# dfm/tinygp

Measured on AMD Instinct MI355X. Metric: GP log_probability evals/sec + Cholesky TFLOP/s (fp64), N=16,384, higher is better.
Workload: dtype f64; 1 GPU; c2: 1.5^2 ExpSquared(2.5), 1-D X, N=16384, fp64, diag=0.01, constant-density synthetic inputs (SURVEY 8d), dense Cholesky + tri-solve; n=16384, d=1, parallelism=single, nb_outer=1024

## Files before the change

tinygp_amd/csrc/capi.hip:

```cpp
#include <cmath>
#include <cstdlib>
#include <chrono>
#include <cstring>
#include <string>

#include "tgp_common.h"
#define CHAIN_HD __host__ __device__
#include "chain_tasks.h"
#define TILE_HD
#include "tile_order.h"

namespace tgp {

static thread_local std::string g_error;

void set_error(const char* fmt, ...) {
  char buf[1024];
  va_list ap;
  va_start(ap, fmt);
  vsnprintf(buf, sizeof(buf), fmt, ap);
  va_end(ap);
  g_error = buf;
}

// ... 147 lines not shown
    const char* b = getenv("TGP_SERIALIZED_KERNELS");
    auto on = [](const char* v) { return v != nullptr && *v && strcmp(v, "0") != 0 && strcasecmp(v, "false") != 0; };
    if (on(a) || on(b)) {
      ctx->serializing_tool = true;
      ctx->chain_polls = 0;
    }
  }
  TGP_HIP_TRY(hipStreamCreateWithPriority(&ctx->panel_stream, hipStreamNonBlocking, hi));
  TGP_HIP_TRY(hipStreamCreateWithPriority(&ctx->update_stream, hipStreamNonBlocking, hi));
  TGP_HIP_TRY(hipStreamCreateWithPriority(&ctx->asm_stream, hipStreamNonBlocking, lo));
  TGP_HIP_TRY(hipEventCreateWithFlags(&ctx->ev_asm, hipEventDisableTiming));
  TGP_HIP_TRY(hipEventCreateWithFlags(&ctx->ev_d, hipEventDisableTiming));
  TGP_HIP_TRY(hipEventCreateWithFlags(&ctx->ev_e, hipEventDisableTiming));
  TGP_HIP_TRY(hipEventCreateWithFlags(&ctx->ev_f, hipEventDisableTiming));
  TGP_HIP_TRY(hipEventCreateWithFlags(&ctx->ev_g1, hipEventDisableTiming));
  TGP_HIP_TRY(hipEventCreateWithFlags(&ctx->ev_g2, hipEventDisableTiming));
  TGP_HIP_TRY(hipEventCreateWithFlags(&ctx->ev_h, hipEventDisableTiming));
  TGP_HIP_TRY(hipEventCreateWithFlags(&ctx->ev_i, hipEventDisableTiming));
  TGP_HIP_TRY(hipEventCreateWithFlags(&ctx->ev_j, hipEventDisableTiming));
  TGP_HIP_TRY(hipEventCreateWithFlags(&ctx->ev_c, hipEventDisableTiming));
  TGP_HIP_TRY(hipEventCreateWithFlags(&ctx->ev_join, hipEventDisableTiming));
  TGP_HIP_TRY(hipEventCreateWithFlags(&ctx->ev_a, hipEventDisableTiming));
  TGP_HIP_TRY(hipEventCreateWithFlags(&ctx->ev_b, hipEventDisableTiming));
  TGP_HIP_TRY(hipMalloc(&ctx->d_scal, 16 * sizeof(double)));
  TGP_HIP_TRY(hipMalloc(&ctx->d_info, sizeof(int32_t)));
  TGP_HIP_TRY(hipMalloc(&ctx->d_step_flag, 64));
  TGP_HIP_TRY(hipMemset(ctx->d_step_flag, 0, 64));
  TGP_HIP_TRY(hipMalloc(&ctx->d_chain_flags, size_t(tgp::CHAIN_MAX_ROW_TILES) * 64 * sizeof(uint32_t)));
  TGP_HIP_TRY(hipMemset(ctx->d_chain_flags, 0, size_t(tgp::CHAIN_MAX_ROW_TILES) * 64 * sizeof(uint32_t)));
  TGP_HIP_TRY(hipMalloc(&ctx->d_chain_ticket, 4096));
  TGP_HIP_TRY(hipMemset(ctx->d_chain_ticket, 0, 4096));
  TGP_HIP_TRY(hipMalloc(&ctx->d_chain_red, size_t(2) * CHAIN_MAX_ROW_TILES * sizeof(double)));
  hipDeviceProp_t prop;
  TGP_HIP_TRY(hipGetDeviceProperties(&prop, device));
  ctx->cus = prop.multiProcessorCount;
  *out = ctx;
  return TGP_OK;
}

int tgp_ctx_destroy(tgp_ctx* ctx) {
  if (!ctx) return TGP_OK;
  hipSetDevice(ctx->device);
  hipStreamSynchronize(ctx->stream);
  if (ctx->panel_stream) hipStreamSynchronize(ctx->panel_stream);
  if (ctx->solve_stream) {
    hipStreamSynchronize(ctx->solve_stream);
    hipStreamDestroy(ctx->solve_stream);
  }
  if (ctx->ev_c) hipEventDestroy(ctx->ev_c);
  if (ctx->ev_join) hipEventDestroy(ctx->ev_join);
  if (ctx->ev_asm_gate) hipEventDestroy(ctx->ev_asm_gate);
  if (ctx->rescue_stream) hipStreamDestroy(ctx->rescue_stream);
  if (ctx->update_stream) {
    hipStreamSynchronize(ctx->update_stream);
    hipStreamDestroy(ctx->update_stream);
  }
  if (ctx->asm_stream) {
    hipStreamSynchronize(ctx->asm_stream);
    hipStreamDestroy(ctx->asm_stream);
  }
  if (ctx->ev_asm) hipEventDestroy(ctx->ev_asm);
  if (ctx->ev_d) hipEventDestroy(ctx->ev_d);
  if (ctx->ev_e) hipEventDestroy(ctx->ev_e);
  if (ctx->ev_f) hipEventDestroy(ctx->ev_f);
  if (ctx->ev_g1) hipEventDestroy(ctx->ev_g1);
  if (ctx->ev_g2) hipEventDestroy(ctx->ev_g2);
  if (ctx->ev_h) hipEventDestroy(ctx->ev_h);
  if (ctx->ev_i) hipEventDestroy(ctx->ev_i);
  if (ctx->ev_j) hipEventDestroy(ctx->ev_j);
  for (auto e : ctx->ev_pool) hipEventDestroy(e);
  if (ctx->ev_a) hipEventDestroy(ctx->ev_a);
  if (ctx->ev_b) hipEventDestroy(ctx->ev_b);
  if (ctx->d_scal) hipFree(ctx->d_scal);
  if (ctx->d_info) hipFree(ctx->d_info);
  if (ctx->d_step_flag) hipFree(ctx->d_step_flag);
  if (ctx->d_chain_flags) hipFree(ctx->d_chain_flags);
  if (ctx->d_chain_ticket) hipFree(ctx->d_chain_ticket);
  if (ctx->d_chain_red) hipFree(ctx->d_chain_red);
  if (ctx->d_chain_stamps) hipFree(ctx->d_chain_stamps);
  for (auto& kv : ctx->chain_tables)
    if (kv.second.dev) hipFree(kv.second.dev);
  if (ctx->d_dinv) hipFree(ctx->d_dinv);
  if (ctx->d_work) hipFree(ctx->d_work);
  if (ctx->d_gemm_ws) hipFree(ctx->d_gemm_ws);
  if (ctx->panel_stream) hipStreamDestroy(ctx->panel_stream);
  if (ctx->own_stream && ctx->stream) hipStreamDestroy(ctx->stream);
  delete ctx;
  return TGP_OK;
}

int tgp_ctx_sync(tgp_ctx* ctx) {
  CTX_GUARD(ctx);
  TGP_HIP_TRY(hipStreamSynchronize(ctx->stream));
  return TGP_OK;
}

static int64_t* option_slot(tgp_ctx* ctx, const char* key) {
// ... 39 lines not shown
  if (!strcmp(key, "host_join")) return &ctx->host_join;
  if (!strcmp(key, "late_join")) return &ctx->late_join;
  if (!strcmp(key, "chain_reduce")) return &ctx->chain_reduce;
  if (!strcmp(key, "asm_defer")) return &ctx->asm_defer;
  if (!strcmp(key, "tile_band")) return &ctx->tile_band;
  if (!strcmp(key, "fault_inject")) return &ctx->fault_inject;
  if (!strcmp(key, "poll_timeout_ms")) return &ctx->poll_timeout_ms;
  if (!strcmp(key, "timeout_retries")) return &ctx->timeout_retries;
  return nullptr;
}

static int set_option_checked(tgp_ctx* ctx, const char* key, int64_t value, int64_t* old) {
  int64_t* slot = option_slot(ctx, key);
  TGP_ARG_CHECK(slot != nullptr, "unknown option '%s'", key);
  if (slot == &ctx->nb_outer)
    TGP_ARG_CHECK(value >= TILE && value % TILE == 0, "nb_outer must be a positive multiple of %d", TILE);
  if (slot == &ctx->sub_panel || slot == &ctx->nb_first)
    TGP_ARG_CHECK(value >= 0 && value % TILE == 0, "%s must be a multiple of %d (0: off)", key, TILE);
  if (slot == &ctx->chain_batch) TGP_ARG_CHECK(value >= 0 && value <= 32, "chain_batch must be in [0, 32]");
  if (slot == &ctx->chain_batch_lag) TGP_ARG_CHECK(value >= 1 && value <= 64, "chain_batch_lag must be in [1, 64]");
  if (slot == &ctx->chain_batch_minrows) TGP_ARG_CHECK(value >= 0 && value <= 4096, "chain_batch_minrows must be in [0, 4096]");
  if (slot == &ctx->chain_batch_rowlag) TGP_ARG_CHECK(value >= 2 && value <= 4096, "chain_batch_rowlag must be in [2, 4096]");
  if (old) *old = *slot;
  if (slot == &ctx->poll_timeout_ms && ctx->has_device) return set_poll_limit(ctx, value);
  *slot = value;
  return TGP_OK;
}

int tgp_ctx_set_option(tgp_ctx* ctx, const char* key, int64_t value, int64_t* old) {
  TGP_ARG_CHECK(ctx != nullptr && key != nullptr, "null argument");
  return set_option_checked(ctx, key, value, old);
}

int tgp_ctx_get_option(tgp_ctx* ctx, const char* key, int64_t* value) {
  TGP_ARG_CHECK(ctx != nullptr && key != nullptr && value != nullptr, "null argument");
  int64_t* slot = option_slot(ctx, key);
  TGP_ARG_CHECK(slot != nullptr, "unknown option '%s'", key);
  if (slot == &ctx->poll_timeout_ms && ctx->has_device) ctx->poll_timeout_ms = tgp::poll_limit_ms();
  *value = *slot;
  return TGP_OK;
}

static int apply_options(tgp_ctx* ctx, const char* options) {
  if (options == nullptr) return TGP_OK;
  std::string all(options);
  size_t pos = 0;
// ... 346 lines not shown
                                 hipMemcpyHostToDevice, ctx->stream));
      TGP_TRY(launch_set_lower_from_rowmajor<T>(ctx, s->n, s->npad, (const T*)s->scratch, A, s->npad));
    } else {
      TGP_TRY(assemble_lower<T>(ctx, s->kp, s->n, s->d, (const T*)s->X, (const T*)s->diag, A, s->npad));
    }
    if (prof) TGP_HIP_TRY(hipEventRecord(e1, ctx->stream));
    int32_t inf = 0;
    ctx->defer_join = ctx->late_join != 0;
    ctx->join_deferred = false;
    reductions_begin(ctx, s->npad, fused != 0);
    int st = potrf<T>(ctx, s->npad, A, s->npad, (T*)s->dinv, &inf, fused ? (T*)s->vec : (T*)nullptr);
    ctx->defer_join = false;
    const bool reduce = reductions_end(ctx);
    if (st < 0) return st;
    s->info = inf;
    if (prof) TGP_HIP_TRY(hipEventRecord(e2, ctx->stream));
    if (reduce) {
      TGP_TRY(launch_sum_log_diag<T>(ctx, s->n, A, s->npad, 1));
      if (fused) TGP_TRY(launch_sum_squares<T>(ctx, s->n, (const T*)s->vec, 0));
    }
    return TGP_OK;
  });
  if (status < 0) return status;
  double two[2] = {0, 0};
  int32_t inf_late = 0;
  const bool late = ctx->join_deferred;
  ctx->join_deferred = false;
  TGP_HIP_TRY(hipMemcpyAsync(two, ctx->d_scal, 2 * sizeof(double), hipMemcpyDeviceToHost, ctx->stream));
  if (late) TGP_HIP_TRY(hipMemcpyAsync(&inf_late, ctx->d_info, sizeof(int32_t), hipMemcpyDeviceToHost, ctx->stream));
  TGP_HIP_TRY(hipStreamSynchronize(ctx->stream));
  if (late) {
    if (inf_late == INT32_MIN) {
      tgp::set_error("potrf: a device-side hand-off did not arrive within poll_timeout_ms (a lost or starved chain launch)");
      if (prof) { hipEventDestroy(e0); hipEventDestroy(e1); hipEventDestroy(e2); }
      return TGP_E_TIMEOUT;
    }
    s->info = inf_late;
  }
  s->ms[5] = std::chrono::duration<double, std::milli>(ctx->submitted - host0).count();
  s->logdet_half = two[1];
  if (fused && logprob)
    *logprob = -0.5 * two[0] - (s->logdet_half + 0.5 * double(s->n) * std::log(2.0 * M_PI));
  if (prof) {
    float a = 0, b = 0;
    TGP_HIP_TRY(hipEventElapsedTime(&a, e0, e1));
    TGP_HIP_TRY(hipEventElapsedTime(&b, e1, e2));
    s->ms[0] = a;
    s->ms[1] = b;
    s->ms[2] = ctx->prof_syrk_ms;
    s->ms[3] = (double)ctx->prof_syrk_launches;
    s->ms[6] = ctx->prof_syrk_flops;
    s->ms[7] = ctx->prof_syrk_union_ms;
    hipEventDestroy(e0);
    hipEventDestroy(e1);
// ... 554 lines not shown
```

tinygp_amd/csrc/chol.hip:

```cpp
#include <algorithm>
#include <atomic>
#include <functional>
#include <type_traits>

#include <thread>

#include "tgp_common.h"
#define CHAIN_HD __host__ __device__
#include "chain_tasks.h"

namespace tgp {

namespace {

typedef double d4 __attribute__((ext_vector_type(4)));
typedef float f4 __attribute__((ext_vector_type(4)));

template <typename T> struct Mfma;
template <> struct Mfma<double> {
  using acc_t = d4;
  static __device__ __forceinline__ acc_t mma(double a, double b, acc_t c) {
    return __builtin_amdgcn_mfma_f64_16x16x4f64(a, b, c, 0, 0, 0);
  }
  static __device__ __forceinline__ int drow(int lane, int r) { return (lane >> 4) + 4 * r; }
// ... 298 lines not shown
template <typename T> struct AgentBits;
template <> struct AgentBits<double> { using t = unsigned long long; };
template <> struct AgentBits<float> { using t = unsigned int; };
template <typename T>
__device__ __forceinline__ void st_agent(T* p, T v) {
  typename AgentBits<T>::t b;
  __builtin_memcpy(&b, &v, sizeof(T));
  __hip_atomic_store(reinterpret_cast<typename AgentBits<T>::t*>(p), b, __ATOMIC_RELAXED, __HIP_MEMORY_SCOPE_AGENT);
}

__device__ __forceinline__ void chain_stamp(long long* st, int k) {
  if (st != nullptr && threadIdx.x == 0) st[4 + k] = (long long)__builtin_amdgcn_s_memrealtime();
}

constexpr int CHAIN_FLAG_LD = 64;
constexpr uint32_t CHAIN_FINAL = 127;
constexpr int CHAIN_COLCNT_OFF = 16;
constexpr int CHAIN_QCNT_OFF = 96;
constexpr int CHAIN_XSTEP_OFF = 160;
constexpr int CHAIN_ZFLAG_OFF = 224;
constexpr int CHAIN_YSTATE_OFF = 288;
constexpr int CHAIN_TICKET_WORDS = CHAIN_YSTATE_OFF + int(CHAIN_MAX_ROW_TILES) / CHAIN_FWD_GROUP;
constexpr int CHAIN_PREFIX_OFF = CHAIN_TICKET_WORDS + 16;

template <typename T>
struct ChainArgs {
  T* A0;
  int64_t ld;
  T* dinv;
  int32_t* info;
  uint32_t* flags;
  int32_t* ticket;
  uint32_t epoch32;
  int32_t pivot_base;
  int32_t R;
  int32_t nblk;
  int32_t cb, ce;
  long long* stamps;
  int32_t launch;
  int32_t fast_update;
  const uint64_t* tasks;
  T* y;
  int32_t fgs;
  int32_t fprev;
  double* red;
  double* scal;
  int32_t red_total;
};

template <int NAP>
__device__ __forceinline__ void chain_wait(const uint32_t* f0, uint32_t v0, const uint32_t* f1, uint32_t v1,
                                           const uint32_t* f2, uint32_t v2, int32_t* info) {
  if (threadIdx.x < 64) {
    const int lane = threadIdx.x;
    const uint32_t* f = lane == 0 ? f0 : (lane == 1 ? f1 : (lane == 2 ? f2 : nullptr));
// ... 10 lines not shown
      ++spin;
      if (__any(dead)) {
        if (lane == 0) atomicExch(info, STEP_TIMEOUT);
        break;
      }
    }
    if (lane == 0) __builtin_amdgcn_fence(__ATOMIC_ACQUIRE, "agent");
  }
  __syncthreads();
}

__device__ __forceinline__ void chain_publish(uint32_t* word, uint32_t value, int32_t* colcnt = nullptr) {
  asm volatile("s_waitcnt vmcnt(0)" ::: "memory");
  __syncthreads();
  if (threadIdx.x == 0) {
    __hip_atomic_store(word, value, __ATOMIC_RELAXED, __HIP_MEMORY_SCOPE_AGENT);
    if (colcnt != nullptr) __hip_atomic_fetch_add(colcnt, 1, __ATOMIC_RELAXED, __HIP_MEMORY_SCOPE_AGENT);
  }
}

__device__ void potf2_prefix_wait(const int32_t* count, int32_t target, int32_t* info) {
  PollClock clk;
  for (unsigned spin = 0;; ++spin) {
    if (__hip_atomic_load(count, __ATOMIC_RELAXED, __HIP_MEMORY_SCOPE_AGENT) >= target) break;
    __builtin_amdgcn_s_sleep(8);
    if ((spin & 255) == 255 && (clk.expired(spin) || poisoned(info))) {
      atomicExch(info, STEP_TIMEOUT);
      break;
    }
  }
  __builtin_amdgcn_fence(__ATOMIC_ACQUIRE, "agent");
}

__global__ __launch_bounds__(64) void chain_poll_kernel(const int32_t* __restrict__ count, int32_t target,
                                                        int32_t* __restrict__ info) {
  if (threadIdx.x != 0) return;
  PollClock clk;
  for (unsigned spin = 0;; ++spin) {
    if (__hip_atomic_load(count, __ATOMIC_RELAXED, __HIP_MEMORY_SCOPE_AGENT) >= target) break;
    __builtin_amdgcn_s_sleep(16);
    if ((spin & 255) == 255 && (clk.expired(spin) || poisoned(info))) {
      atomicExch(info, STEP_TIMEOUT);
      break;
    }
  }
}

template <typename T, int PARTS>
__device__ __forceinline__ void chain_update_full(const ChainArgs<T>& q, T* S, int i, int c, int k, int part) {
  static_assert(PARTS == 1 || PARTS == 4 || PARTS == 8, "whole tile, row quarters or row eighths");
  using M = Mfma<T>;
  using acc_t = typename M::acc_t;
  typedef T T2 __attribute__((ext_vector_type(2)));
  const int tid = threadIdx.x, lane = tid & 63;
  const int w = __builtin_amdgcn_readfirstlane(tid >> 6);
  const int lrow = lane & 15, lk = lane >> 4;
  const int64_t ld = q.ld;
  constexpr int FK = 16, F_LD = 144;
  static_assert(4 * FK * F_LD == 36 * 256, "the operand buffers are exactly potf2's tile image");
  T* sA = S;
  T* sB = S + 2 * FK * F_LD;
  const int rbase = PARTS == 1 ? (w >> 1) * 32 : (PARTS == 4 ? part * 32 : part * 16);
// ... 728 lines not shown
#define CHAIN_WAVES_PER_EU(T) (sizeof(T) == 8 ? 4 : 3)
#endif
template <typename T>
__global__ __launch_bounds__(512) __attribute__((amdgpu_waves_per_eu(CHAIN_WAVES_PER_EU(T), 4))) void chain_kernel(const ChainArgs<T> q) {
  __shared__ __attribute__((aligned(16))) T S[36 * 256];
  __shared__ T Rs[2 * 16];
  __shared__ T Dg[256];
  __shared__ int s_task[7];
  using acc_t = typename Mfma<T>::acc_t;
  if (threadIdx.x == 0) {
    const int t = atomicAdd(q.ticket, 1);
    s_task[4] = t;
    const ChainTask task = chain_unpack(q.tasks[t]);
    const int kind = task.kind, ti = task.i, tc = task.c, tk = task.k;
    s_task[5] = task.part;
    s_task[6] = task.k0;
    s_task[0] = kind; s_task[1] = ti; s_task[2] = tc; s_task[3] = tk;
  }
  __syncthreads();
  const int kind = __builtin_amdgcn_readfirstlane(s_task[0]);
  const int ti = __builtin_amdgcn_readfirstlane(s_task[1]);
  const int tc = __builtin_amdgcn_readfirstlane(s_task[2]);
  const int tk = __builtin_amdgcn_readfirstlane(s_task[3]);
  if (kind > 8) return;
  long long* st = nullptr;
  if (q.stamps != nullptr) {
    st = q.stamps + int64_t(__builtin_amdgcn_readfirstlane(s_task[4])) * 16;
    if (threadIdx.x == 0) {
      st[0] = kind; st[1] = kind == 1 ? tc : ti; st[2] = tc; st[3] = q.launch | (tk << 8) | (s_task[6] << 16);
      for (int k = 1; k < 12; ++k) st[4 + k] = 0;
    }
    chain_stamp(st, 0);
  }
  const uint32_t E = q.epoch32;
  const bool head_final = q.cb == 0;
  if (kind == 7) {
    const int c = tc;
    const int g = c / q.fgs;
    const bool prev = c > 0 || q.fprev != 0;
    chain_wait_counts(c - 1 > q.cb ? q.ticket + CHAIN_YSTATE_OFF + g : nullptr, c - 1 - q.cb,
                      (c == 0 && head_final) ? nullptr : reinterpret_cast<const int32_t*>(q.flags + c * CHAIN_FLAG_LD + c),
                      int32_t(E + CHAIN_FINAL), c > q.cb ? q.ticket + CHAIN_ZFLAG_OFF + (c - 1) : nullptr, 1, q.info);
    chain_stamp(st, 1);
    chain_fsolve<T>(q, S, c, prev);
    chain_stamp(st, 2);
    asm volatile("s_waitcnt vmcnt(0)" ::: "memory");
// ... 767 lines not shown

int join_bounded(tgp_ctx* ctx, hipStream_t st, int64_t n) {
  TGP_TRY(ev_record(ctx, ctx->ev_join, st));
  const auto t0 = std::chrono::steady_clock::now();
  const double budget_ms = double(poll_limit_ms()) + 3.0 * (double(n) * double(n) * double(n) / 3.0) / 2e13 * 1e3;
  for (long spin = 0;; ++spin) {
    const hipError_t e = hipEventQuery(ctx->ev_join);
    if (e == hipSuccess) return TGP_OK;
    if (e != hipErrorNotReady) {
      set_error("hipEventQuery failed: %s", hipGetErrorString(e));
      return TGP_E_HIP;
    }
    (void)hipGetLastError();
    if (ctx->fault_inject == 1) {
      ctx->fault_inject = 0;
      break;
    }
    if ((spin & 63) != 63) continue;
    const double ms = std::chrono::duration<double, std::milli>(std::chrono::steady_clock::now() - t0).count();
    if (ms > budget_ms) break;
    if (ms > 50.0) std::this_thread::sleep_for(std::chrono::microseconds(200));
  }
  if (ctx->rescue_stream == nullptr) TGP_HIP_TRY(hipStreamCreateWithFlags(&ctx->rescue_stream, hipStreamNonBlocking));
  for (int c = 0; c < CHAIN_FLAG_LD; ++c)
    (void)hipStreamWriteValue32(ctx->rescue_stream, ctx->d_chain_ticket + CHAIN_COLCNT_OFF + c, 0x7fffffffu, 0);
  for (hipStream_t q : {ctx->rescue_stream, ctx->asm_stream, ctx->panel_stream, ctx->update_stream, ctx->solve_stream, ctx->stream})
    if (q) (void)hipStreamSynchronize(q);
  (void)hipGetLastError();
  set_error("potrf: the followers of a chain launch were still waiting after %.0f ms (stream wait-values released by the host)", budget_ms);
  return TGP_E_TIMEOUT;
}

template <typename T>
int launch_potf2(tgp_ctx* ctx, hipStream_t st, T* A, int64_t ld, T* dinv, int32_t* info,
                 int32_t pivot_base, const T* Xp, int64_t ldx) {
  if (ctx->trace) {
    trace_push(ctx, 1, st, trace_off(ctx, A), trace_off(ctx, Xp), ld);
    return TGP_OK;
  }
  const int32_t* wc = ctx->potf2_wait_counter;
  const int32_t wt = (int32_t)ctx->potf2_wait_target;
  ctx->potf2_wait_counter = nullptr;
  if (Xp != nullptr)
    hipLaunchKernelGGL((potf2_kernel<T, true>), dim3(1), dim3(512), 0, st, A, ld, dinv, info, pivot_base, Xp, ldx, wc, wt);
  else
    hipLaunchKernelGGL((potf2_kernel<T, false>), dim3(1), dim3(512), 0, st, A, ld, dinv, info, pivot_base, Xp, ldx, wc, wt);
  TGP_HIP_TRY(hipGetLastError());
  return TGP_OK;
}

template <typename T>
int launch_trsm(tgp_ctx* ctx, hipStream_t st, int64_t m, const T* L, int64_t ldl, const T* dinv,
                T* B, int64_t ldb) {
  if (m == 0) return TGP_OK;
  TGP_ARG_CHECK(m % 16 == 0, "trsm: m must be a multiple of 16");
  if (ctx->trace) {
    trace_push(ctx, 2, st, trace_off(ctx, L), trace_off(ctx, B), m, ldl);
    return TGP_OK;
  }
  hipLaunchKernelGGL((trsm_kernel<T>), dim3((unsigned)((m + 63) / 64)), dim3(256), 0, st, m, L,
                     ldl, dinv, B, ldb);
  TGP_HIP_TRY(hipGetLastError());
  return TGP_OK;
}
// ... 58 lines not shown
  auto found = ctx->chain_tables.find(key);
  if (found == ctx->chain_tables.end()) {
    const std::vector<ChainTask> list = chain_build((int)R, (int)nblk, (int)cb, (int)ce, pol, fwd, CHAIN_FWD_GROUP);
    tgp_ctx::ChainTable tab;
    tab.count = (int64_t)list.size();
    if (tab.count > 0) {
      std::vector<uint64_t> words(list.size());
      for (size_t u = 0; u < list.size(); ++u) words[u] = chain_pack(list[u]);
      TGP_HIP_TRY(hipMalloc((void**)&tab.dev, words.size() * sizeof(uint64_t)));
      TGP_HIP_TRY(hipMemcpy(tab.dev, words.data(), words.size() * sizeof(uint64_t), hipMemcpyHostToDevice));
    }
    found = ctx->chain_tables.emplace(key, tab).first;
  }
  const int64_t tasks = found->second.count;
  if (tasks == 0) {
    if (counters_ready != nullptr) TGP_TRY(ev_record(ctx, counters_ready, st));
    return TGP_OK;
  }
  ctx->step_epoch = (ctx->step_epoch + 1) & 0x1FFFFFFu;
  if (ctx->step_epoch == 0) ctx->step_epoch = 1;
  const uint32_t epoch = ctx->step_epoch;
  ChainArgs<T> q;
  q.A0 = A0; q.ld = ld; q.dinv = dinv0; q.info = ctx->d_info; q.flags = ctx->d_chain_flags;
  q.ticket = ctx->d_chain_ticket; q.epoch32 = epoch * 128u; q.pivot_base = (int32_t)pivot_base; q.R = (int32_t)R;
  q.nblk = (int32_t)nblk;
  q.cb = (int32_t)cb; q.ce = (int32_t)ce;
  q.stamps = nullptr;
  q.launch = (int32_t)ctx->chain_launches++;
  q.fast_update = (int32_t)ctx->chain_fast_update;
  q.tasks = found->second.dev;
  q.y = y0;
  q.fgs = CHAIN_FWD_GROUP;
  q.fprev = fprev ? 1 : 0;
  q.red = red != 0 ? ctx->d_chain_red : nullptr;
  q.scal = red != 0 ? ctx->d_scal : nullptr;
  q.red_total = red == 2 ? (int32_t)ctx->chain_red_total : 0;
  if (ctx->chain_stamps != 0 && ctx->chain_stamp_base + tasks <= CHAIN_STAMP_TASKS) {
    if (ctx->d_chain_stamps == nullptr)
      TGP_HIP_TRY(hipMalloc((void**)&ctx->d_chain_stamps, size_t(CHAIN_STAMP_TASKS) * 16 * sizeof(long long)));
    q.stamps = ctx->d_chain_stamps + ctx->chain_stamp_base * 16;
    ctx->chain_stamp_base += tasks;
  }
  TGP_HIP_TRY(hipMemsetAsync(ctx->d_chain_ticket, 0, size_t(CHAIN_TICKET_WORDS) * sizeof(int32_t), st));
  if (counters_ready != nullptr) TGP_TRY(ev_record(ctx, counters_ready, st));
  const size_t dyn = ctx->chain_lds_pad > 0 ? size_t(ctx->chain_lds_pad) + (sizeof(T) == 4 ? 36 * 256 * 4 : 0) : 0;
  hipLaunchKernelGGL((chain_kernel<T>), dim3((unsigned)tasks), dim3(512), dyn, st, q);
  TGP_HIP_TRY(hipGetLastError());
  return TGP_OK;
}

int launch_chain_poll(tgp_ctx* ctx, hipStream_t st, const void* A0, int64_t ld, int64_t R, int64_t c, bool first_external) {
  if (ctx->trace) {
    trace_push(ctx, 12, st, trace_off(ctx, static_cast<const double*>(A0)), ld, c);
    return TGP_OK;
  }
  const int32_t target = (int32_t)(R - c - ((c == 0 && first_external) ? 1 : 0));
  int32_t* count = ctx->d_chain_ticket + CHAIN_COLCNT_OFF + c;
  if (ctx->chain_polls == 3 && ctx->can_wait_value) {
    ctx->wait_values_inflight = true;
    TGP_HIP_TRY(hipStreamWaitValue32(st, count, (uint32_t)target, hipStreamWaitValueGte, 0xffffffffu));
    return TGP_OK;
  }
  hipLaunchKernelGGL(chain_poll_kernel, dim3(1), dim3(64), 0, st, count, target, ctx->d_info);
  TGP_HIP_TRY(hipGetLastError());
  return TGP_OK;
}

int launch_prefix_poll(tgp_ctx* ctx, hipStream_t st, const int32_t* counter, int64_t target, int64_t c_off, int64_t ld) {
  if (ctx->trace) {
    trace_push(ctx, 13, st, c_off, ld);
    return TGP_OK;
  }
  hipLaunchKernelGGL(chain_poll_kernel, dim3(1), dim3(64), 0, st, counter, (int32_t)target, ctx->d_info);
  TGP_HIP_TRY(hipGetLastError());
  return TGP_OK;
}

template <typename T>
int compute_dinv(tgp_ctx* ctx, int64_t n, const T* L, int64_t ld, T* dinv) {
  if (n == 0) return TGP_OK;
  hipLaunchKernelGGL((dinv_kernel<T>), dim3((unsigned)((n + 255) / 256)), dim3(256), 0,
                     ctx->stream, n, L, ld, dinv);
  TGP_HIP_TRY(hipGetLastError());
  return TGP_OK;
}

template <typename T>
int launch_trsv_fwd_step(tgp_ctx* ctx, hipStream_t st, int64_t m_below, const T* Ljj, int64_t ld,
                         const T* dj, T* yj) {
  if (ctx->trace) {
    trace_push(ctx, 4, st, trace_off(ctx, Ljj), m_below, ld);
    return TGP_OK;
  }
  hipLaunchKernelGGL((trsv_diag_fwd_kernel<T>), dim3(1), dim3(128), 0, st, Ljj, ld, dj, yj);
  if (m_below > 0)
    hipLaunchKernelGGL((trsv_update_fwd_kernel<T>), dim3((unsigned)((m_below + 255) / 256)),
// ... 144 lines not shown
  }
  return TGP_OK;
}

template <typename T>
int potrf(tgp_ctx* ctx, int64_t n, T* A, int64_t ld, T* dinv, int32_t* info_host, T* y) {
  TGP_ARG_CHECK(n % TILE == 0 && ld >= n, "potrf: n must be a multiple of %d and ld >= n", TILE);
  if (info_host) *info_host = 0;
  if (n == 0) return TGP_OK;
  ctx->potf2_wait_counter = nullptr;
  ctx->prefix_hint_cols = 0;
  ctx->prefix_hint_counter = nullptr;
  ctx->reserve_hint = 0;
  hipStream_t S0 = ctx->stream, S1 = ctx->panel_stream;
  if (ctx->solve_on_update == 0 && y != nullptr) TGP_TRY(ensure_solve_stream(ctx));
  hipStream_t S2 = ctx->solve_on_update != 0 ? ctx->update_stream : ctx->solve_stream;
  if (y != nullptr) {
    TGP_TRY(ev_record(ctx, ctx->ev_c, S0));
    TGP_TRY(st_wait(ctx, S2, ctx->ev_c));
  }
  int64_t NB = ctx->nb_outer;
  if (NB < TILE) NB = TILE;
  NB = NB / TILE * TILE;
  if (!ctx->trace) TGP_HIP_TRY(hipMemsetAsync(ctx->d_info, 0, sizeof(int32_t), S0));
  ctx->chain_stamp_base = 0;
  ctx->chain_launches = 0;
  ctx->chain_polls_pending = false;
  const bool prof_on = ctx->profile != 0 && !ctx->trace;
  std::vector<ProfSpan> spans;
  ctx->ev_used = 0;
  hipEvent_t prof_t0 = nullptr;
  const bool span_dump = prof_on && getenv("TGP_SPAN_DUMP") != nullptr;
  if (prof_on) {
    TGP_TRY(prof_event(ctx, &prof_t0));
    TGP_HIP_TRY(hipEventRecord(prof_t0, S0));
  }

  auto potf2_at = [&](hipStream_t st, int64_t j0, bool pend) -> int {
    return panel_potf2<T>(ctx, st, A, ld, dinv, 0, j0, pend);
  };
  auto panel = [&](hipStream_t st, int64_t k0, int64_t kb, bool head_done, int64_t after_blocks,
                   const std::function<int(hipEvent_t)>& mid) -> int {
    return panel_chain<T>(ctx, st, n, A, ld, dinv, 0, k0, kb, head_done, y, after_blocks, mid);
  };
  const std::function<int(hipEvent_t)> no_mid = [](hipEvent_t) { return TGP_OK; };
  auto trailing = [&](hipStream_t sq, int64_t m, int64_t nn, int64_t kb, const T* P, T* C, int role) -> int {
    ProfSpan sp{};
// ... 53 lines not shown
    for (int64_t k0 = 0; k0 < n; k0 += width(k0)) s0.push_back(k0);
    s0.push_back(n);
    const int64_t P = (int64_t)s0.size() - 1;
    hipEvent_t ev_chain[2] = {ctx->ev_b, ctx->ev_g1}, ev_pfx[2] = {ctx->ev_g2, ctx->ev_e}, ev_T[2] = {ctx->ev_i, ctx->ev_j};
    const bool asm_side = ctx->asm_pending;
    ctx->asm_pending = false;
    if (P == 1 && !asm_side) {
      TGP_TRY(panel(S0, 0, s0[1] - s0[0], false, 0, no_mid));
      TGP_TRY(run_deferred_asm(ctx, nullptr));
    } else {
    TGP_TRY(ev_record(ctx, ctx->ev_a, S0));
    TGP_TRY(st_wait(ctx, S1, ctx->ev_a));
    TGP_TRY(panel(S1, 0, s0[1] - s0[0], false, 0, no_mid));
    TGP_TRY(run_deferred_asm(ctx, nullptr));
    TGP_TRY(ev_record(ctx, ev_chain[0], S1));
    for (int64_t p = 0; p + 1 < P; ++p) {
      const int64_t kb = s0[p + 1] - s0[p], next = s0[p + 1], wn = s0[p + 2] - s0[p + 1], mt = n - next;
      const T* Pp = A + s0[p] * ld + next;
      T* C = A + next * ld + next;
      TGP_TRY(st_wait(ctx, S0, ev_chain[p & 1]));
      if (p == 0 && asm_side) TGP_TRY(st_wait(ctx, S0, ctx->ev_asm));
      const bool prefix = wn < mt && ctx->chain_polls != 0;
      int32_t* counter = ctx->d_chain_ticket + CHAIN_PREFIX_OFF + (p & 3);
      if (prefix) {
        if (!ctx->trace) TGP_HIP_TRY(hipMemsetAsync(counter, 0, sizeof(int32_t), S0));
        TGP_TRY(ev_record(ctx, ev_pfx[p & 1], S0));
        ctx->prefix_hint_cols = wn;
        ctx->prefix_hint_counter = counter;
      }
      const int64_t t = mt / TILE;
      if (t * (t + 1) / 2 <= ctx->reserve_max_tiles) ctx->reserve_hint = ctx->chain_reserve;
      TGP_TRY(trailing(S0, mt, mt, kb, Pp, C, 0));
      if (!prefix) TGP_TRY(ev_record(ctx, ev_T[p & 1], S0));
      if (prefix) {
        const int64_t tm = mt / TILE, tp = wn / TILE;
        TGP_TRY(st_wait(ctx, S1, ev_pfx[p & 1]));
        if (ctx->trace || ctx->chain_polls == 2) {
          TGP_TRY(launch_prefix_poll(ctx, S1, counter, tp * tm - tp * (tp - 1) / 2, trace_off(ctx, C), ld));
        } else {
          ctx->potf2_wait_counter = counter;
          ctx->potf2_wait_target = tp * tm - tp * (tp - 1) / 2;
        }
      } else {
        TGP_TRY(st_wait(ctx, S1, ev_T[p & 1]));
      }
      if (p == 0 && asm_side) TGP_TRY(st_wait(ctx, S1, ctx->ev_asm));
      TGP_TRY(potf2_at(S1, next, false));
      TGP_TRY(chain_of_panel(S1, next, wn));
      TGP_TRY(ev_record(ctx, ev_chain[(p + 1) & 1], S1));
    }
    TGP_TRY(st_wait(ctx, S0, ev_chain[(P - 1) & 1]));
    }
  } else
  if (la && ctx->chain_kernel != 0 && ctx->chain_depth2 != 0) {
    std::vector<int64_t> s0;
    for (int64_t k0 = 0; k0 < n; k0 += width(k0)) s0.push_back(k0);
    s0.push_back(n);
    const int64_t P = (int64_t)s0.size() - 1;
    hipEvent_t ev_chain[2] = {ctx->ev_b, ctx->ev_g1}, ev_pre[2] = {ctx->ev_g2, ctx->ev_e};
    auto first_role = [&](int64_t m, int64_t nn) -> int {
      const int64_t tiles = (m / TILE) * (nn / TILE) - (nn / TILE) * (nn / TILE - 1) / 2;
      return tiles <= ctx->first_small_tiles ? 4 : 0;
    };
    const bool asm_side = ctx->asm_pending;
// ... 144 lines not shown
    }
  }
  if (y != nullptr) {
    TGP_TRY(ev_record(ctx, ctx->ev_c, S2));
    TGP_TRY(st_wait(ctx, S0, ctx->ev_c));
  }
  int32_t info = 0;
  ctx->submitted = std::chrono::steady_clock::now();
  if (ctx->defer_join && !ctx->trace && !prof_on && !(ctx->wait_values_inflight && ctx->host_join != 0)) {
    ctx->wait_values_inflight = false;
    ctx->join_deferred = true;
    if (info_host) *info_host = 0;
    return TGP_OK;
  }
  if (!ctx->trace) {
    TGP_HIP_TRY(hipMemcpyAsync(&info, ctx->d_info, sizeof(int32_t), hipMemcpyDeviceToHost, S0));
    if (ctx->wait_values_inflight && ctx->host_join != 0) {
      ctx->wait_values_inflight = false;
      TGP_TRY(join_bounded(ctx, S0, n));
    } else {
      ctx->wait_values_inflight = false;
      TGP_HIP_TRY(hipStreamSynchronize(S0));
    }
  }
  if (prof_on) {
    ctx->prof_syrk_ms = 0;
    ctx->prof_syrk_flops = 0;
    ctx->prof_syrk_union_ms = 0;
    ctx->prof_syrk_launches = (int64_t)spans.size();
    std::vector<std::pair<double, double>> iv;
    for (auto& sp : spans) {
      float ms = 0, at = 0;
      TGP_HIP_TRY(hipEventElapsedTime(&ms, sp.e0, sp.e1));
      TGP_HIP_TRY(hipEventElapsedTime(&at, prof_t0, sp.e0));
      ctx->prof_syrk_ms += ms;
      ctx->prof_syrk_flops += sp.flops;
      iv.emplace_back(double(at), double(at) + double(ms));
      if (span_dump)
        fprintf(stderr, "span at %8.3f ms  + %7.3f ms  %8.2f GF  %5.1f TF/s\n", at, ms, sp.flops * 1e-9, sp.flops / ms * 1e-9);
    }
    std::sort(iv.begin(), iv.end());
    double hi = -1e300;
    for (const auto& q : iv) {
      if (q.first > hi) {
        ctx->prof_syrk_union_ms += q.second - q.first;
        hi = q.second;
// ... 253 lines not shown
```

tinygp_amd/csrc/dist.hip:

```cpp
#include <cmath>

#include "tgp_common.h"

using namespace tgp;

struct tgp_dist {
  tgp_ctx* ctx = nullptr;
  int dtype = TGP_F64;
  int64_t n = 0, npad = 0, nb = 0, nblk = 0, nloc = 0;
  int d = 1, G = 1, rank = 0;
  void* X = nullptr;
  void* diag = nullptr;
  void* A = nullptr;
  void* dinv = nullptr;
  static constexpr int NSLOT = 3;
  void* ring[3] = {nullptr, nullptr, nullptr};
  hipEvent_t ev_solve[3] = {nullptr, nullptr, nullptr};
  bool ev_solve_set[3] = {false, false, false};
  hipEvent_t ev_arrived = nullptr;
  hipEvent_t ev_rest[3] = {nullptr, nullptr, nullptr};
  bool ev_rest_set[3] = {false, false, false};
  hipEvent_t ev_pre[2] = {nullptr, nullptr};
  bool ev_pre_set[2] = {false, false};
  hipEvent_t ev_asm_done = nullptr;
// ... 335 lines not shown
    for (int64_t l = 0; l < h->nloc; ++l) {
      const int64_t j0 = (l * h->G + h->rank) * h->nb;
      const int64_t n1 = std::max<int64_t>(h->n - j0, 0), n2 = std::max<int64_t>(std::min(h->nb, h->n - j0), 0);
      T* Ab = (T*)h->A + l * h->nb * h->npad + j0;
      TGP_HIP_TRY(hipMemset2DAsync(Ab, size_t(h->npad) * es, 0, size_t(h->npad - j0) * es, size_t(h->nb), ctx->stream));
      if (n1 > 0 && n2 > 0)
        TGP_HIP_TRY(hipMemcpy2DAsync(Ab, size_t(h->npad) * es, (const char*)K_host + (size_t(j0) * h->n + size_t(j0)) * es,
                                     size_t(h->n) * es, size_t(n1) * es, size_t(n2), hipMemcpyHostToDevice, ctx->stream));
      if (n2 < h->nb)
        hipLaunchKernelGGL((pad_identity_kernel<T>), dim3((unsigned)((h->nb - n2 + 255) / 256)), dim3(256), 0, ctx->stream, Ab,
                           h->npad, n2, h->nb);
    }
    TGP_HIP_TRY(hipGetLastError());
    TGP_HIP_TRY(hipStreamSynchronize(ctx->stream));
    return TGP_OK;
  });
}

int tgp_dist_begin(tgp_dist* h, const void* resid_host) {
  DIST_GUARD(h);
  tgp_ctx* ctx = h->ctx;
  const size_t es = esz(h->dtype);
  TGP_HIP_TRY(hipMemsetAsync(ctx->d_info, 0, sizeof(int32_t), ctx->stream));
  TGP_HIP_TRY(hipMemsetAsync(h->d_logdet, 0, size_t(h->nblk + 1) * sizeof(double), ctx->stream));
  h->solving = resid_host != nullptr;
  if (h->solving) {
    TGP_HIP_TRY(hipMemcpyAsync(h->x, resid_host, size_t(h->n) * es, hipMemcpyHostToDevice, ctx->stream));
    if (h->npad > h->n)
      TGP_HIP_TRY(hipMemsetAsync((char*)h->x + size_t(h->n) * es, 0, size_t(h->npad - h->n) * es, ctx->stream));
  }
  for (bool& b : h->ev_solve_set) b = false;
  for (bool& b : h->ev_rest_set) b = false;
  for (bool& b : h->ev_pre_set) b = false;
  h->s1_saw_asm = false;
  return TGP_OK;
}

int tgp_dist_first_panel(tgp_dist* h) {
  DIST_GUARD(h);
  return ddispatch(h->dtype, [&](auto tag) {
    using T = decltype(tag);
    if (h->asm_deferred) {
      h->asm_deferred = false;
      TGP_TRY(assemble_columns<T>(h, 1, h->nloc));
    }
    TGP_HIP_TRY(hipEventRecord(h->ev_asm_done, h->ctx->stream));
// ... 589 lines not shown
```

tinygp_amd/csrc/tgp_common.h:

```cpp
#pragma once

#include <hip/hip_runtime.h>

#include <cstdarg>
#include <cstdint>
#include <cstdio>
#include <chrono>
#include <array>
#include <functional>
#include <map>
#include <mutex>
#include <vector>

#include "../../include/tgp_hip.h"

namespace tgp {

constexpr int TILE = TGP_TILE;
constexpr int SUB = 16;

void set_error(const char* fmt, ...);

#define TGP_HIP_TRY(expr)                                                                  \
  do {                                                                                     \
    hipError_t _e = (expr);                                                                \
    if (_e != hipSuccess) {                                                                \
      ::tgp::set_error("%s failed: %s (%s:%d)", #expr, hipGetErrorString(_e), __FILE__,    \
                       __LINE__);                                                          \
      return (_e == hipErrorOutOfMemory) ? TGP_E_NOMEM : TGP_E_HIP;                        \
    }                                                                                      \
  } while (0)

#define TGP_ARG_CHECK(cond, ...)        \
  do {                                  \
    if (!(cond)) {                      \
      ::tgp::set_error(__VA_ARGS__);    \
      return TGP_E_ARG;                 \
// ... 63 lines not shown
  int64_t sub_panel = 0;
  int64_t sub_panel_min_rows = 0;
  int64_t nb_first = 0;
  int64_t split_tail = 0;
  int64_t gemm_role = 1;
  int64_t late_join = 1;
  int64_t chain_reduce = 1;
  double* d_chain_red = nullptr;
  int64_t chain_red_total = 0;
  int64_t chain_red_written = 0;
  bool reductions_done = false;
  bool defer_join = false;
  bool join_deferred = false;
  int64_t reserve_hint = 0;
  int64_t prefix_hint_cols = 0;
  int32_t* prefix_hint_counter = nullptr;
  const int32_t* potf2_wait_counter = nullptr;
  int64_t potf2_wait_target = 0;
  uint32_t* d_step_flag = nullptr;
  uint32_t step_epoch = 0;
  int64_t chain_kernel = 1;
  uint32_t* d_chain_flags = nullptr;
  int32_t* d_chain_ticket = nullptr;
  int64_t chain_fast_update = 0;
  int64_t chain_batch = 1;
  int64_t chain_batch_lag = 1;
  int64_t chain_batch_rowlag = 4;
  int64_t chain_batch_minrows = 32;
  struct ChainTable {
    uint64_t* dev = nullptr;
    int64_t count = 0;
  };
  std::map<std::array<int64_t, 9>, ChainTable> chain_tables;
  int64_t chain_full_rows = 4096;
  int64_t chain_depth2 = 1;
  int64_t chain_merged = 1;
  int64_t chain_sub_panel = 0;
  int64_t chain_sub_min_rows = 0;
  int64_t chain_sub_role = 4;
  int64_t kmat_plain_div = 0;
  int64_t chain_polls = 1;
  int64_t chain_fwd_tasks = 1;
  bool chain_fwd_now = false;
  bool wait_values_inflight = false;
  int64_t tile_band = 8;
  int64_t asm_defer = 0;
  std::function<int()> deferred_asm;
  hipEvent_t ev_asm_gate = nullptr;
  int64_t fault_inject = 0;
  int64_t host_join = 1;
  bool serializing_tool = false;
  hipStream_t rescue_stream = nullptr;
  hipEvent_t ev_join = nullptr;
  bool has_device = false;
  bool can_wait_value = false;
  int64_t poll_timeout_ms = 4000;
  int64_t timeout_retries = 0;
  int64_t chain_pre_wait = 0;
  int64_t chain_gate_split = 0;
  int64_t chain_lds_pad = 10240;
  int64_t chain_stamps = 0;
  long long* d_chain_stamps = nullptr;
  int64_t chain_stamp_base = 0;
  int64_t chain_launches = 0;
  bool chain_polls_pending = false;
  double* d_scal = nullptr;
  int32_t* d_info = nullptr;
  void* d_dinv = nullptr;
  size_t dinv_bytes = 0;
  void* d_gemm_ws = nullptr;
  size_t gemm_ws_bytes = 0;
  void* d_work = nullptr;
  size_t work_bytes = 0;
  std::vector<hipEvent_t> ev_pool;
  size_t ev_used = 0;
  double prof_syrk_ms = 0, prof_syrk_flops = 0, prof_syrk_union_ms = 0;
  int64_t prof_syrk_launches = 0;
  int cus = 0;
  std::vector<tgp_trace_rec>* trace = nullptr;
  const void* trace_base = nullptr;
};

namespace tgp {

inline int64_t trace_stream_id(const tgp_ctx* ctx, hipStream_t st) {
  if (st == ctx->stream) return 0;
  if (st == ctx->panel_stream) return 1;
  if (st == ctx->solve_stream) return 2;
  if (st == ctx->update_stream) return 3;
  if (st == ctx->asm_stream) return 4;
// ... 92 lines not shown

template <typename T>
int launch_gemm_tri(tgp_ctx* ctx, hipStream_t st, int64_t m, int64_t n, int64_t k, const T* A, int64_t lda,
                    const T* B, int64_t ldb, T* C, int64_t ldc, int lower, int mode, int batch, int64_t sA,
                    int64_t sB, int64_t sC);

template <typename T>
int launch_gemm_nt_dist(tgp_ctx* ctx, hipStream_t st, int64_t n_rows, int64_t nb, int64_t k,
                        const T* P, int64_t ldp, T* Cloc, int64_t ldc, int G, int rank, int64_t l0,
                        int64_t nloc, int64_t reserve = 0);

template <typename T>
int launch_potf2(tgp_ctx* ctx, hipStream_t st, T* A, int64_t ld, T* dinv, int32_t* info,
                 int32_t pivot_base, const T* Xp = nullptr, int64_t ldx = 0);
template <typename T>
int launch_trsm(tgp_ctx* ctx, hipStream_t st, int64_t m, const T* L, int64_t ldl, const T* dinv,
                T* B, int64_t ldb);
template <typename T>
int launch_panel_step(tgp_ctx* ctx, hipStream_t st, int64_t m, T* Ljj, int64_t ld, T* dj, int32_t* info,
                      int32_t pivot_base, const T* Xp, bool has_p);

constexpr int64_t CHAIN_MAX_ROW_TILES = 4096;
constexpr int64_t CHAIN_STAMP_TASKS = 32768;
template <typename T>
int launch_chain(tgp_ctx* ctx, hipStream_t st, T* A0, int64_t ld, T* dinv0, int64_t pivot_base, int64_t R,
                 int64_t nblk, int64_t cb, int64_t ce, bool head_done, hipEvent_t counters_ready = nullptr,
                 T* y0 = nullptr, bool fprev = false);
int launch_chain_poll(tgp_ctx* ctx, hipStream_t st, const void* A0, int64_t ld, int64_t R, int64_t c, bool first_external);
int launch_prefix_poll(tgp_ctx* ctx, hipStream_t st, const int32_t* counter, int64_t target, int64_t c_off, int64_t ld);
int set_poll_limit(tgp_ctx* ctx, int64_t ms);
int64_t poll_limit_ms();
int join_bounded(tgp_ctx* ctx, hipStream_t st, int64_t n);
int run_deferred_asm(tgp_ctx* ctx, hipStream_t behind);
template <typename T>
int panel_potf2(tgp_ctx* ctx, hipStream_t st, T* A, int64_t ld, T* dinv, int64_t pivot_off,
                int64_t j0, bool pend);
template <typename T>
int panel_chain(tgp_ctx* ctx, hipStream_t st, int64_t n, T* A, int64_t ld, T* dinv,
                int64_t pivot_off, int64_t k0, int64_t kb, bool head_done, T* y,
                int64_t after_blocks, const std::function<int(hipEvent_t)>& mid, int64_t blk_begin = 0,
                int64_t blk_end = -1);
template <typename T>
int launch_trsv_fwd_step(tgp_ctx* ctx, hipStream_t st, int64_t m_below, const T* Ljj, int64_t ld,
                         const T* dj, T* yj);
template <typename T>
int potrf(tgp_ctx* ctx, int64_t n, T* A, int64_t ld, T* dinv, int32_t* info_host, T* y = nullptr);
// ... 58 lines not shown
```

Before: 39.89 evals/s.

## Replace per-launch counter memsets with monotonic counters and double-buffered chain tickets

Drops the memset of the chain ticket block before every chain launch and the prefix-counter memsets. Prefix counters become monotonic, with host-tracked cumulative targets and wrap-safe comparisons. Chain tickets alternate between two blocks, and the running kernel zeroes the other block for the next launch. The info word and result scalars are merged into one device record copied into pinned host memory with a single memcpy. This removes many small memset nodes and one copy from the critical path, at the cost of more complex state tracking and clean/dirty bookkeeping.

Measured after the change: 39.91 evals/s (median of 2 runs). No clear change (+0.0%).

```diff
diff --git a/tinygp_amd/csrc/capi.hip b/tinygp_amd/csrc/capi.hip
--- a/tinygp_amd/csrc/capi.hip
+++ b/tinygp_amd/csrc/capi.hip
@@ -193,14 +193,23 @@
   TGP_HIP_TRY(hipEventCreateWithFlags(&ctx->ev_join, hipEventDisableTiming));
   TGP_HIP_TRY(hipEventCreateWithFlags(&ctx->ev_a, hipEventDisableTiming));
   TGP_HIP_TRY(hipEventCreateWithFlags(&ctx->ev_b, hipEventDisableTiming));
-  TGP_HIP_TRY(hipMalloc(&ctx->d_scal, 16 * sizeof(double)));
-  TGP_HIP_TRY(hipMalloc(&ctx->d_info, sizeof(int32_t)));
+  {
+    void* rec = nullptr;
+    TGP_HIP_TRY(hipMalloc(&rec, 17 * sizeof(double)));
+    TGP_HIP_TRY(hipMemset(rec, 0, 17 * sizeof(double)));
+    ctx->d_info = static_cast<int32_t*>(rec);
+    ctx->d_scal = static_cast<double*>(rec) + 1;
+    static_assert(sizeof(tgp_ctx::ResultRecord) == 3 * sizeof(double), "info | scal[0] | scal[1]");
+    TGP_HIP_TRY(hipHostMalloc((void**)&ctx->h_record, sizeof(tgp_ctx::ResultRecord), hipHostMallocDefault));
+  }
   TGP_HIP_TRY(hipMalloc(&ctx->d_step_flag, 64));
   TGP_HIP_TRY(hipMemset(ctx->d_step_flag, 0, 64));
   TGP_HIP_TRY(hipMalloc(&ctx->d_chain_flags, size_t(tgp::CHAIN_MAX_ROW_TILES) * 64 * sizeof(uint32_t)));
   TGP_HIP_TRY(hipMemset(ctx->d_chain_flags, 0, size_t(tgp::CHAIN_MAX_ROW_TILES) * 64 * sizeof(uint32_t)));
-  TGP_HIP_TRY(hipMalloc(&ctx->d_chain_ticket, 4096));
-  TGP_HIP_TRY(hipMemset(ctx->d_chain_ticket, 0, 4096));
+  TGP_HIP_TRY(hipMalloc(&ctx->d_chain_ticket, tgp::CHAIN_COUNTER_BYTES));
+  TGP_HIP_TRY(hipMemset(ctx->d_chain_ticket, 0, tgp::CHAIN_COUNTER_BYTES));
+  ctx->counters.reset();
+  ctx->counters.clean = true;
   TGP_HIP_TRY(hipMalloc(&ctx->d_chain_red, size_t(2) * CHAIN_MAX_ROW_TILES * sizeof(double)));
   hipDeviceProp_t prop;
   TGP_HIP_TRY(hipGetDeviceProperties(&prop, device));
@@ -242,8 +251,8 @@
   for (auto e : ctx->ev_pool) hipEventDestroy(e);
   if (ctx->ev_a) hipEventDestroy(ctx->ev_a);
   if (ctx->ev_b) hipEventDestroy(ctx->ev_b);
-  if (ctx->d_scal) hipFree(ctx->d_scal);
   if (ctx->d_info) hipFree(ctx->d_info);
+  if (ctx->h_record) hipHostFree(ctx->h_record);
   if (ctx->d_step_flag) hipFree(ctx->d_step_flag);
   if (ctx->d_chain_flags) hipFree(ctx->d_chain_flags);
   if (ctx->d_chain_ticket) hipFree(ctx->d_chain_ticket);
@@ -329,6 +338,7 @@
   if (slot == &ctx->chain_batch_minrows) TGP_ARG_CHECK(value >= 0 && value <= 4096, "chain_batch_minrows must be in [0, 4096]");
   if (slot == &ctx->chain_batch_rowlag) TGP_ARG_CHECK(value >= 2 && value <= 4096, "chain_batch_rowlag must be in [2, 4096]");
   if (old) *old = *slot;
+  if (*slot != value) ctx->counters.clean = false;
   if (slot == &ctx->poll_timeout_ms && ctx->has_device) return set_poll_limit(ctx, value);
   *slot = value;
   return TGP_OK;
@@ -721,14 +731,15 @@
     return TGP_OK;
   });
   if (status < 0) return status;
-  double two[2] = {0, 0};
-  int32_t inf_late = 0;
   const bool late = ctx->join_deferred;
   ctx->join_deferred = false;
-  TGP_HIP_TRY(hipMemcpyAsync(two, ctx->d_scal, 2 * sizeof(double), hipMemcpyDeviceToHost, ctx->stream));
-  if (late) TGP_HIP_TRY(hipMemcpyAsync(&inf_late, ctx->d_info, sizeof(int32_t), hipMemcpyDeviceToHost, ctx->stream));
+  tgp_ctx::ResultRecord* rec = ctx->h_record;
+  TGP_HIP_TRY(hipMemcpyAsync(rec, ctx->d_info, sizeof(*rec), hipMemcpyDeviceToHost, ctx->stream));
   TGP_HIP_TRY(hipStreamSynchronize(ctx->stream));
+  const double two[2] = {rec->scal[0], rec->scal[1]};
+  const int32_t inf_late = rec->info;
   if (late) {
+    tgp::counters_commit(ctx, inf_late);
     if (inf_late == INT32_MIN) {
       tgp::set_error("potrf: a device-side hand-off did not arrive within poll_timeout_ms (a lost or starved chain launch)");
       if (prof) { hipEventDestroy(e0); hipEventDestroy(e1); hipEventDestroy(e2); }
diff --git a/tinygp_amd/csrc/chol.hip b/tinygp_amd/csrc/chol.hip
--- a/tinygp_amd/csrc/chol.hip
+++ b/tinygp_amd/csrc/chol.hip
@@ -344,6 +344,7 @@
 constexpr int CHAIN_YSTATE_OFF = 288;
 constexpr int CHAIN_TICKET_WORDS = CHAIN_YSTATE_OFF + int(CHAIN_MAX_ROW_TILES) / CHAIN_FWD_GROUP;
 constexpr int CHAIN_PREFIX_OFF = CHAIN_TICKET_WORDS + 16;
+static_assert(CHAIN_PREFIX_OFF + CounterBook::PREFIX_WORDS <= CHAIN_BLOCK_STRIDE, "the prefix counters sit inside block 0's stride");
 
 template <typename T>
 struct ChainArgs {
@@ -353,6 +354,7 @@
   int32_t* info;
   uint32_t* flags;
   int32_t* ticket;
+  int32_t* ticket_next;
   uint32_t epoch32;
   int32_t pivot_base;
   int32_t R;
@@ -409,7 +411,7 @@
 __device__ void potf2_prefix_wait(const int32_t* count, int32_t target, int32_t* info) {
   PollClock clk;
   for (unsigned spin = 0;; ++spin) {
-    if (__hip_atomic_load(count, __ATOMIC_RELAXED, __HIP_MEMORY_SCOPE_AGENT) >= target) break;
+    if (counter_reached((uint32_t)__hip_atomic_load(count, __ATOMIC_RELAXED, __HIP_MEMORY_SCOPE_AGENT), (uint32_t)target)) break;
     __builtin_amdgcn_s_sleep(8);
     if ((spin & 255) == 255 && (clk.expired(spin) || poisoned(info))) {
       atomicExch(info, STEP_TIMEOUT);
@@ -424,7 +426,7 @@
   if (threadIdx.x != 0) return;
   PollClock clk;
   for (unsigned spin = 0;; ++spin) {
-    if (__hip_atomic_load(count, __ATOMIC_RELAXED, __HIP_MEMORY_SCOPE_AGENT) >= target) break;
+    if (counter_reached((uint32_t)__hip_atomic_load(count, __ATOMIC_RELAXED, __HIP_MEMORY_SCOPE_AGENT), (uint32_t)target)) break;
     __builtin_amdgcn_s_sleep(16);
     if ((spin & 255) == 255 && (clk.expired(spin) || poisoned(info))) {
       atomicExch(info, STEP_TIMEOUT);
@@ -1199,6 +1201,9 @@
   const int ti = __builtin_amdgcn_readfirstlane(s_task[1]);
   const int tc = __builtin_amdgcn_readfirstlane(s_task[2]);
   const int tk = __builtin_amdgcn_readfirstlane(s_task[3]);
+  if (__builtin_amdgcn_readfirstlane(s_task[4]) == 0)
+    for (int w = threadIdx.x; w < CHAIN_TICKET_WORDS; w += 512)
+      __hip_atomic_store(q.ticket_next + w, 0, __ATOMIC_RELAXED, __HIP_MEMORY_SCOPE_AGENT);
   if (kind > 8) return;
   long long* st = nullptr;
   if (q.stamps != nullptr) {
@@ -2012,8 +2017,10 @@
     if (ms > 50.0) std::this_thread::sleep_for(std::chrono::microseconds(200));
   }
   if (ctx->rescue_stream == nullptr) TGP_HIP_TRY(hipStreamCreateWithFlags(&ctx->rescue_stream, hipStreamNonBlocking));
-  for (int c = 0; c < CHAIN_FLAG_LD; ++c)
-    (void)hipStreamWriteValue32(ctx->rescue_stream, ctx->d_chain_ticket + CHAIN_COLCNT_OFF + c, 0x7fffffffu, 0);
+  for (int b = 0; b < 2; ++b)
+    for (int c = 0; c < CHAIN_FLAG_LD; ++c)
+      (void)hipStreamWriteValue32(ctx->rescue_stream, ctx->d_chain_ticket + b * CHAIN_BLOCK_STRIDE + CHAIN_COLCNT_OFF + c,
+                                  0x7fffffffu, 0);
   for (hipStream_t q : {ctx->rescue_stream, ctx->asm_stream, ctx->panel_stream, ctx->update_stream, ctx->solve_stream, ctx->stream})
     if (q) (void)hipStreamSynchronize(q);
   (void)hipGetLastError();
@@ -2021,6 +2028,16 @@
   return TGP_E_TIMEOUT;
 }
 
+int counters_begin(tgp_ctx* ctx, hipStream_t st) {
+  if (!ctx->counters.clean) {
+    TGP_HIP_TRY(hipMemsetAsync(ctx->d_chain_ticket, 0, CHAIN_COUNTER_BYTES, st));
+    TGP_HIP_TRY(hipMemsetAsync(ctx->d_info, 0, sizeof(int32_t), st));
+    ctx->counters.reset();
+  }
+  ctx->counters.clean = false;
+  return TGP_OK;
+}
+
 template <typename T>
 int launch_potf2(tgp_ctx* ctx, hipStream_t st, T* A, int64_t ld, T* dinv, int32_t* info,
                  int32_t pivot_base, const T* Xp, int64_t ldx) {
@@ -2029,7 +2046,7 @@
     return TGP_OK;
   }
   const int32_t* wc = ctx->potf2_wait_counter;
-  const int32_t wt = (int32_t)ctx->potf2_wait_target;
+  const int32_t wt = (int32_t)(uint32_t)ctx->potf2_wait_target;
   ctx->potf2_wait_counter = nullptr;
   if (Xp != nullptr)
     hipLaunchKernelGGL((potf2_kernel<T, true>), dim3(1), dim3(512), 0, st, A, ld, dinv, info, pivot_base, Xp, ldx, wc, wt);
@@ -2134,7 +2151,14 @@
   const uint32_t epoch = ctx->step_epoch;
   ChainArgs<T> q;
   q.A0 = A0; q.ld = ld; q.dinv = dinv0; q.info = ctx->d_info; q.flags = ctx->d_chain_flags;
-  q.ticket = ctx->d_chain_ticket; q.epoch32 = epoch * 128u; q.pivot_base = (int32_t)pivot_base; q.R = (int32_t)R;
+  if (!ctx->counters_armed) {
+    TGP_HIP_TRY(hipMemsetAsync(ctx->d_chain_ticket, 0, CHAIN_COUNTER_BYTES, st));
+    ctx->counters.reset();
+    ctx->counters.clean = false;
+  }
+  const uint32_t blk = ctx->counters.take_chain_block();
+  ctx->chain_ticket_cur = ctx->d_chain_ticket + blk * CHAIN_BLOCK_STRIDE;
+  q.ticket = ctx->chain_ticket_cur; q.ticket_next = ctx->d_chain_ticket + (blk ^ 1u) * CHAIN_BLOCK_STRIDE; q.epoch32 = epoch * 128u; q.pivot_base = (int32_t)pivot_base; q.R = (int32_t)R;
   q.nblk = (int32_t)nblk;
   q.cb = (int32_t)cb; q.ce = (int32_t)ce;
   q.stamps = nullptr;
@@ -2153,7 +2177,6 @@
     q.stamps = ctx->d_chain_stamps + ctx->chain_stamp_base * 16;
     ctx->chain_stamp_base += tasks;
   }
-  TGP_HIP_TRY(hipMemsetAsync(ctx->d_chain_ticket, 0, size_t(CHAIN_TICKET_WORDS) * sizeof(int32_t), st));
   if (counters_ready != nullptr) TGP_TRY(ev_record(ctx, counters_ready, st));
   const size_t dyn = ctx->chain_lds_pad > 0 ? size_t(ctx->chain_lds_pad) + (sizeof(T) == 4 ? 36 * 256 * 4 : 0) : 0;
   hipLaunchKernelGGL((chain_kernel<T>), dim3((unsigned)tasks), dim3(512), dyn, st, q);
@@ -2167,7 +2190,7 @@
     return TGP_OK;
   }
   const int32_t target = (int32_t)(R - c - ((c == 0 && first_external) ? 1 : 0));
-  int32_t* count = ctx->d_chain_ticket + CHAIN_COLCNT_OFF + c;
+  int32_t* count = (ctx->chain_ticket_cur != nullptr ? ctx->chain_ticket_cur : ctx->d_chain_ticket) + CHAIN_COLCNT_OFF + c;
   if (ctx->chain_polls == 3 && ctx->can_wait_value) {
     ctx->wait_values_inflight = true;
     TGP_HIP_TRY(hipStreamWaitValue32(st, count, (uint32_t)target, hipStreamWaitValueGte, 0xffffffffu));
@@ -2183,7 +2206,7 @@
     trace_push(ctx, 13, st, c_off, ld);
     return TGP_OK;
   }
-  hipLaunchKernelGGL(chain_poll_kernel, dim3(1), dim3(64), 0, st, counter, (int32_t)target, ctx->d_info);
+  hipLaunchKernelGGL(chain_poll_kernel, dim3(1), dim3(64), 0, st, counter, (int32_t)(uint32_t)target, ctx->d_info);
   TGP_HIP_TRY(hipGetLastError());
   return TGP_OK;
 }
@@ -2374,7 +2397,14 @@
   int64_t NB = ctx->nb_outer;
   if (NB < TILE) NB = TILE;
   NB = NB / TILE * TILE;
-  if (!ctx->trace) TGP_HIP_TRY(hipMemsetAsync(ctx->d_info, 0, sizeof(int32_t), S0));
+  struct Armed {
+    tgp_ctx* c;
+    ~Armed() { c->counters_armed = false; }
+  } armed{ctx};
+  if (!ctx->trace) {
+    TGP_TRY(counters_begin(ctx, S0));
+    ctx->counters_armed = true;
+  }
   ctx->chain_stamp_base = 0;
   ctx->chain_launches = 0;
   ctx->chain_polls_pending = false;
@@ -2474,8 +2504,9 @@
       if (p == 0 && asm_side) TGP_TRY(st_wait(ctx, S0, ctx->ev_asm));
       const bool prefix = wn < mt && ctx->chain_polls != 0;
       int32_t* counter = ctx->d_chain_ticket + CHAIN_PREFIX_OFF + (p & 3);
+      const int64_t pfx_tiles = (wn / TILE) * (mt / TILE) - (wn / TILE) * (wn / TILE - 1) / 2;
+      const int64_t pfx_target = prefix && !ctx->trace ? (int64_t)ctx->counters.prefix_target(int(p & 3), (uint32_t)pfx_tiles) : pfx_tiles;
       if (prefix) {
-        if (!ctx->trace) TGP_HIP_TRY(hipMemsetAsync(counter, 0, sizeof(int32_t), S0));
         TGP_TRY(ev_record(ctx, ev_pfx[p & 1], S0));
         ctx->prefix_hint_cols = wn;
         ctx->prefix_hint_counter = counter;
@@ -2485,13 +2516,12 @@
       TGP_TRY(trailing(S0, mt, mt, kb, Pp, C, 0));
       if (!prefix) TGP_TRY(ev_record(ctx, ev_T[p & 1], S0));
       if (prefix) {
-        const int64_t tm = mt / TILE, tp = wn / TILE;
         TGP_TRY(st_wait(ctx, S1, ev_pfx[p & 1]));
         if (ctx->trace || ctx->chain_polls == 2) {
-          TGP_TRY(launch_prefix_poll(ctx, S1, counter, tp * tm - tp * (tp - 1) / 2, trace_off(ctx, C), ld));
+          TGP_TRY(launch_prefix_poll(ctx, S1, counter, pfx_target, trace_off(ctx, C), ld));
         } else {
           ctx->potf2_wait_counter = counter;
-          ctx->potf2_wait_target = tp * tm - tp * (tp - 1) / 2;
+          ctx->potf2_wait_target = pfx_target;
         }
       } else {
         TGP_TRY(st_wait(ctx, S1, ev_T[p & 1]));
@@ -2682,6 +2712,7 @@
       ctx->wait_values_inflight = false;
       TGP_HIP_TRY(hipStreamSynchronize(S0));
     }
+    counters_commit(ctx, info);
   }
   if (prof_on) {
     ctx->prof_syrk_ms = 0;
diff --git a/tinygp_amd/csrc/counters.h b/tinygp_amd/csrc/counters.h
--- /dev/null
+++ b/tinygp_amd/csrc/counters.h
@@ -0,0 +1,36 @@
+#pragma once
+#include <cstdint>
+
+#if defined(__HIPCC__) || defined(__CUDACC__)
+#define TGP_COUNTERS_HD __host__ __device__
+#else
+#define TGP_COUNTERS_HD
+#endif
+
+namespace tgp {
+
+TGP_COUNTERS_HD inline bool counter_reached(uint32_t counter, uint32_t target) { return int32_t(counter - target) >= 0; }
+
+struct CounterBook {
+  static constexpr int PREFIX_WORDS = 4;
+  uint32_t prefix_total[PREFIX_WORDS] = {0, 0, 0, 0};
+  uint32_t chain_block = 0;
+  bool clean = false;
+
+  uint32_t prefix_target(int word, uint32_t increments) {
+    uint32_t& t = prefix_total[word & (PREFIX_WORDS - 1)];
+    t += increments;
+    return t;
+  }
+  uint32_t take_chain_block() {
+    const uint32_t b = chain_block;
+    chain_block ^= 1u;
+    return b;
+  }
+  void reset() {
+    for (uint32_t& t : prefix_total) t = 0;
+    chain_block = 0;
+  }
+};
+
+}
diff --git a/tinygp_amd/csrc/dist.hip b/tinygp_amd/csrc/dist.hip
--- a/tinygp_amd/csrc/dist.hip
+++ b/tinygp_amd/csrc/dist.hip
@@ -381,6 +381,7 @@
   tgp_ctx* ctx = h->ctx;
   const size_t es = esz(h->dtype);
   TGP_HIP_TRY(hipMemsetAsync(ctx->d_info, 0, sizeof(int32_t), ctx->stream));
+  ctx->counters.clean = false;
   TGP_HIP_TRY(hipMemsetAsync(h->d_logdet, 0, size_t(h->nblk + 1) * sizeof(double), ctx->stream));
   h->solving = resid_host != nullptr;
   if (h->solving) {
diff --git a/tinygp_amd/csrc/tgp_common.h b/tinygp_amd/csrc/tgp_common.h
--- a/tinygp_amd/csrc/tgp_common.h
+++ b/tinygp_amd/csrc/tgp_common.h
@@ -13,6 +13,7 @@
 #include <vector>
 
 #include "../../include/tgp_hip.h"
+#include "counters.h"
 
 namespace tgp {
 
@@ -122,6 +123,9 @@
   int64_t chain_kernel = 1;
   uint32_t* d_chain_flags = nullptr;
   int32_t* d_chain_ticket = nullptr;
+  int32_t* chain_ticket_cur = nullptr;
+  tgp::CounterBook counters;
+  bool counters_armed = false;
   int64_t chain_fast_update = 0;
   int64_t chain_batch = 1;
   int64_t chain_batch_lag = 1;
@@ -166,6 +170,11 @@
   bool chain_polls_pending = false;
   double* d_scal = nullptr;
   int32_t* d_info = nullptr;
+  struct ResultRecord {
+    int32_t info, pad;
+    double scal[2];
+  };
+  ResultRecord* h_record = nullptr;
   void* d_dinv = nullptr;
   size_t dinv_bytes = 0;
   void* d_gemm_ws = nullptr;
@@ -304,6 +313,10 @@
 
 constexpr int64_t CHAIN_MAX_ROW_TILES = 4096;
 constexpr int64_t CHAIN_STAMP_TASKS = 32768;
+constexpr int64_t CHAIN_BLOCK_STRIDE = 1024;
+constexpr size_t CHAIN_COUNTER_BYTES = size_t(2) * CHAIN_BLOCK_STRIDE * sizeof(int32_t);
+int counters_begin(tgp_ctx* ctx, hipStream_t st);
+inline void counters_commit(tgp_ctx* ctx, int32_t info) { ctx->counters.clean = info == 0; }
 template <typename T>
 int launch_chain(tgp_ctx* ctx, hipStream_t st, T* A0, int64_t ld, T* dinv0, int64_t pivot_base, int64_t R,
                  int64_t nblk, int64_t cb, int64_t ce, bool head_done, hipEvent_t counters_ready = nullptr,
```
